# IXarea/LittleGAN

Hardware: AMD Instinct MI355X
Metric: 128x128 CelebA-shaped images/sec (G+D+Adj step) (higher is better)
Workload: dtype bf16; 1 GPU; C3: 128x128x3 synthetic CelebA, batch 256/GPU, bf16 MFMA conv/transposed-conv + Adjuster branch; global_batch=256, per_gpu_batch=256, image=128, cond_dim=40, parallelism=dp1, launch=eager launches

## Files before the change

littlegan_amd/csrc/conv_down3.hip:

```cpp
#include <type_traits>
#include "lg_internal.h"

namespace {

constexpr int TH = 8, TW = 16;
constexpr int HH = 2 * TH + 3;
constexpr int ROWB = 48;
constexpr int KC = 16;
constexpr int NTAP = 25;
template <bool PAIR>
struct D3L {
  static constexpr int HWH = PAIR ? 10 : 18, HWP = PAIR ? 43 : 2 * HWH;
  static constexpr int NROWS = HH * HWP;
  static constexpr int HB = NROWS * ROWB;
  static constexpr int NPIECE = NROWS * 2;
  static constexpr int PPT = (NPIECE + 255) / 256;
  static constexpr int SRED_OFF = 2 * HB;
  static constexpr int SBIAS_OFF = 2 * HB + 256;
  static constexpr int LDS_BYTES = 2 * HB + 256 + 512;
};
#ifndef LG_D3_DBG
#define LG_D3_DBG 0
#endif
constexpr int DBG = LG_D3_DBG;
constexpr int RING = 10;
constexpr int ADEPTH = 2;
constexpr int STAGGER = 6;
constexpr int BLOCKS_PER_CU = 2;

struct D3Params {
  const __bf16* src;
  const char* wp;
  const float* bias;
  __bf16* out;
  double* spart;
  int B, Hs, Ws, Cs, Hm, Wm, N, N32, KB;
  int tpi_x, tpi, ntn, nitems, nparts;
  LgNormFuse nf;
  const float* nstats;
  float nalpha;
  const __bf16* gsrc;
  const float* bcoef;
  unsigned long long* clk;
};

__device__ __forceinline__ int pix32(int r) {
  const int q = r >> 2, lo = r & 3;
  const int odd = (q ^ (q >> 1) ^ (q >> 2)) & 1;
  const int rank = odd ? ((q == 1) ? 0 : (q == 2) ? 1 : (q == 4) ? 2 : 3) : ((q == 0) ? 0 : (q == 3) ? 1 : (q == 5) ? 2 : 3);
  return odd * 16 + rank * 4 + lo;
}

template <bool PAIR>
constexpr int toff_bytes(int t) {
  return ((t / 5) * D3L<PAIR>::HWP + ((t % 5) >> 1) + ((t % 5) & 1) * D3L<PAIR>::HWH) * ROWB;
}

template <bool STATS, bool FUSE = false, bool PAIR = false, int NW = 128, int NORM = 0>
__global__ __launch_bounds__(256, 2) void conv_down3_kernel(const D3Params p) {
  static_assert(!(STATS && FUSE), "forward moments and backward sums are never needed together");
  static_assert(NORM != 1 || (STATS && NW == 128 && !PAIR), "the normalising form exists for the forward passes with fused moments, 8 x 16 tiles");
  static_assert(NORM != 2 || (!STATS && !PAIR && NW == 64), "the backward-normalising form exists for the 64-column data gradients on 8 x 16 tiles");
  static_assert(NW == 128 || (NW == 64 && !PAIR), "tile widths");
  constexpr int NWV = NW / 32, NI = NW / 32;
  constexpr int PPR = NW / 8, NQ = 128 * PPR / 256;
  using L = D3L<PAIR>;
  constexpr int HWH = L::HWH, HWP = L::HWP, HB = L::HB, NPIECE = L::NPIECE, PPT = L::PPT, SRED_OFF = L::SRED_OFF, SBIAS_OFF = L::SBIAS_OFF;
  extern __shared__ __attribute__((aligned(16))) char smem[];
  double* sred = reinterpret_cast<double*>(smem + SRED_OFF);
  const int tid = threadIdx.x, lane = tid & 63, r = lane & 31, h = lane >> 5;
  const int wid = __builtin_amdgcn_readfirstlane(tid >> 6);
  const int wn = wid % NWV, wm = wid / NWV;
  const int G = gridDim.x;
  const int nchunk = p.Cs / KC;
  const int nx = G < 8 ? G : 8, xcd = (int)blockIdx.x % nx, xidx = (int)blockIdx.x / nx;
  const int lb = lg_xcd_remap(blockIdx.x, G);
  const int nfull = p.nitems / G, nrem = p.nitems - nfull * G;
  const int rcnt = (nrem - xcd + nx - 1) / nx;
  const int rstart = nfull * G + xcd * (nrem / nx) + (xcd < nrem % nx ? xcd : nrem % nx);
  const int nmine = nfull + (xidx < rcnt ? 1 : 0);
  const int total = nmine * nchunk;
  const unsigned long long clk_t0 = __builtin_amdgcn_s_memtime(), clk_r0 = __builtin_amdgcn_s_memrealtime();
  int pl[PPT], pyx[PPT];
#pragma unroll
  for (int u = 0; u < PPT; ++u) {
    const int q = tid + u * 256;
    if constexpr (PAIR) {
      pl[u] = -1; pyx[u] = 0;
      if (q < NPIECE) {
        const int row = q >> 1, hy = row / HWP, hxp = row - hy * HWP;
        pl[u] = row * ROWB + (q & 1) * 16;
        const int sm = hxp >= 24, j2 = hxp - 24 * sm, odd = j2 >= HWH, hx = 2 * (j2 - odd * HWH) + odd;
        pyx[u] = (hxp < 20 || hxp >= 24) && hx < 2 * 8 + 3 ? (hy << 8) | (sm << 7) | hx : (0x7fff << 8);
      }
    } else {
      constexpr int PPROW = 2 * (2 * TW + 3);
      pl[u] = -1; pyx[u] = (0x7fff << 8);
      if (q < HH * PPROW) {
        const int hy = q / PPROW, rem = q - hy * PPROW, hx = rem >> 1;
        const int hxp = (hx & 1) ? HWH + (hx >> 1) : (hx >> 1);
        pl[u] = (hy * HWP + hxp) * ROWB + (rem & 1) * 16;
        pyx[u] = (hy << 8) | hx;
      }
    }
  }
  const int half8 = (tid & 1) * 8;

  int abase[NI];
#pragma unroll
  for (int i = 0; i < NI; ++i) {
    const int m = (wm * NI + i) * 32 + pix32(r);
    const int col = m & 15;
    abase[i] = (2 * (m >> 4) * HWP + (PAIR ? col + 16 * (col >> 3) : col)) * ROWB + h * 16;
  }

  struct Item { int n, y0, x0, tn; };
  auto decode = [&](int k) {
    const int item = k == nfull ? rstart + xidx : lb + k * G;
    Item it;
    it.tn = item % p.ntn;
    const int tm = item / p.ntn;
    if constexpr (PAIR) { it.n = 2 * tm; it.y0 = 0; it.x0 = 0; return it; }
    it.n = tm / p.tpi;
    const int tt = tm - it.n * p.tpi;
    it.y0 = (tt / p.tpi_x) * TH; it.x0 = (tt % p.tpi_x) * TW;
    return it;
  };
  constexpr unsigned OOB = 0x80000000u;
  const int sample_elems = p.Hs * p.Ws * p.Cs;
  unsigned hoff[PPT];
  float nmu0 = 0.f, nml0 = 0.f, nna0 = 0.f, nnb0 = 0.f;
  LgBwdCoef bco{};
  auto set_item = [&](const Item& it) __attribute__((always_inline)) {
    if constexpr (NORM == 1) {
      const lg_const_f32p sp = lg_as_const(p.nstats + (long long)it.n * 8);
      nmu0 = lg_uniform(sp[0]); nna0 = lg_uniform(sp[2]); nnb0 = lg_uniform(sp[3]); nml0 = lg_uniform(sp[4]);
    }
    if constexpr (NORM == 2) {
      const lg_const_f32p sp = lg_as_const(p.bcoef + (long long)it.n * 8);
      bco.mu = lg_uniform(sp[0]); bco.mul = lg_uniform(sp[1]); bco.a = lg_uniform(sp[2]); bco.b = lg_uniform(sp[3]);
      bco.m1 = lg_uniform(sp[4]); bco.m2 = lg_uniform(sp[5]); bco.m1l = lg_uniform(sp[6]); bco.m2l = lg_uniform(sp[7]);
    }
#pragma unroll
    for (int u = 0; u < PPT; ++u) {
      const int sy = 2 * it.y0 - 1 + (pyx[u] >> 8), sx = 2 * it.x0 - 1 + (pyx[u] & (PAIR ? 127 : 255));
      const int sl = PAIR ? (pyx[u] >> 7) & 1 : 0;
      const bool ok = pl[u] >= 0 && (unsigned)sy < (unsigned)p.Hs && (unsigned)sx < (unsigned)p.Ws;
      hoff[u] = ok ? (unsigned)((((sl * p.Hs + sy) * p.Ws + sx) * p.Cs + half8) * 2) : OOB;
    }
  };
  auto issue = [&](const Item& it, int c0, u32x4 (&v)[PPT]) __attribute__((always_inline)) {
    const __amdgpu_buffer_rsrc_t rs = __builtin_amdgcn_make_buffer_rsrc(
        const_cast<__bf16*>(p.src + (long long)it.n * sample_elems), 0, (PAIR ? 2 : 1) * sample_elems * 2, 0x00027000);
#pragma unroll
    for (int u = 0; u < PPT; ++u) v[u] = __builtin_bit_cast(u32x4, __builtin_amdgcn_raw_buffer_load_b128(rs, hoff[u] + (unsigned)c0 * 2u, 0, 0));
  };
  auto issue_g = [&](const Item& it, int c0, u32x4 (&v)[NORM == 2 ? PPT : 1]) __attribute__((always_inline)) {
    if constexpr (NORM == 2) {
      const __amdgpu_buffer_rsrc_t rs = __builtin_amdgcn_make_buffer_rsrc(
          const_cast<__bf16*>(p.gsrc + (long long)it.n * sample_elems), 0, sample_elems * 2, 0x00027000);
#pragma unroll
      for (int u = 0; u < PPT; ++u) v[u] = __builtin_bit_cast(u32x4, __builtin_amdgcn_raw_buffer_load_b128(rs, hoff[u] + (unsigned)c0 * 2u, 0, 0));
    }
  };
  u32x4 gv[NORM == 2 ? PPT : 1];
  auto commit = [&](char* buf, const u32x4 (&v)[PPT]) __attribute__((always_inline)) {
#pragma unroll
    for (int u = 0; u < PPT; ++u)
      if (pl[u] >= 0) {
        u32x4 w = v[u];
        if constexpr (NORM == 2) {
          const u32x4 dn = lg_bwdnorm8(w, gv[u], bco, p.nalpha);
          const bool inside = hoff[u] != OOB;
#pragma unroll
          for (int k = 0; k < 4; ++k) w[k] = inside ? dn[k] : 0u;
        }
        if constexpr (NORM == 1) {
          const u32x4 hn = lg_norm8(w, nmu0, nml0, nna0, nnb0, p.nalpha);
          const bool inside = hoff[u] != OOB;
#pragma unroll
          for (int k = 0; k < 4; ++k) w[k] = inside ? hn[k] : 0u;
        }
        if constexpr ((DBG & 16) != 0) {
          const float mu = p.nf.alpha, mul = 0.001f, na = 1.01f, nb = 0.02f, al = 0.3f;
#pragma unroll
          for (int k = 0; k < 4; ++k) {
            float t0 = __builtin_bit_cast(float, w[k] << 16), t1 = __builtin_bit_cast(float, w[k] & 0xffff0000u);
            t0 = na * ((t0 - mu) - mul) + nb; t1 = na * ((t1 - mu) - mul) + nb;
            t0 = fmaxf(t0, al * t0); t1 = fmaxf(t1, al * t1);
            const __bf16 h0 = (__bf16)t0, h1 = (__bf16)t1;
            const unsigned o = (unsigned)__builtin_bit_cast(unsigned short, h0) | ((unsigned)__builtin_bit_cast(unsigned short, h1) << 16);
            w[k] = pyx[u] != (0x7fff << 8) ? o : 0u;
          }
        }
        *reinterpret_cast<u32x4*>(buf + pl[u]) = w;
      }
  };
  const unsigned lane16 = lane * 16;
  const unsigned wstride = (unsigned)p.N32 * (unsigned)p.KB * 1024u;
  auto wbase = [&](int tn, int kb) {
    return p.wp + ((long long)(tn * NWV + wn) * p.KB + kb) * 1024;
  };
  auto wfrag = [&](const char* base, int t) {
    return *reinterpret_cast<const u32x4*>((base + (unsigned long long)t * wstride) + lane16);
  };

  f32x16 acc[NI];
#pragma unroll
  for (int i = 0; i < NI; ++i)
#pragma unroll
    for (int e = 0; e < 16; ++e) acc[i][e] = 0.f;
  static_assert(NTAP % RING != 0, "the slice body is instantiated for the two ring offsets 0 and NTAP % RING");
  constexpr int AD = ADEPTH;
  u32x4 bf[RING];
  u32x4 hv[PPT];

  Item cur = decode(0);
  set_item(cur);
  issue(cur, 0, hv);
  issue_g(cur, 0, gv);
#pragma unroll
  for (int t = 0; t < RING; ++t) bf[t] = wfrag(wbase(cur.tn, 0), t);
  commit(smem, hv);
  __syncthreads();

  float* sbias = reinterpret_cast<float*>(smem + SBIAS_OFF);
  auto load_bias = [&](int tn) {
    if (tid < NW) sbias[tid] = p.bias ? p.bias[tn * NW + tid] : 0.f;
  };
  load_bias(cur.tn);
  {
    if ((int)blockIdx.x >= (G + 1) / 2)
      for (int i = 0; i < STAGGER; ++i) __builtin_amdgcn_s_sleep(16);
  }
  int k = 0, c = 0;
  auto slice = [&](auto off_c, int s) {
    constexpr int OFF = decltype(off_c)::value;
    const bool more = s + 1 < total;
    const bool last_c = c + 1 == nchunk;
    Item nxt = cur;
    int c2 = c + 1;
    if (last_c) { c2 = 0; if (more) { nxt = decode(k + 1); set_item(nxt); } }
    if (!more) c2 = c;
    if constexpr (!(DBG & 4)) { issue(nxt, c2 * KC, hv); issue_g(nxt, c2 * KC, gv); }
    const char* hbuf = smem + (s & 1) * HB;
    const char* wcur = wbase(cur.tn, c);
    const char* wnxt = wbase(nxt.tn, c2);
    bf16x8 a[AD][NI];
#pragma unroll
    for (int d = 0; d + 1 < AD; ++d)
#pragma unroll
      for (int i = 0; i < NI; ++i) a[d][i] = *reinterpret_cast<const bf16x8*>(hbuf + abase[i] + toff_bytes<PAIR>(d));
    __builtin_amdgcn_sched_barrier(0);
#pragma unroll
    for (int t = 0; t < NTAP; ++t) {
      if (t + AD - 1 < NTAP) {
#pragma unroll
        for (int i = 0; i < NI; ++i)
          a[(t + AD - 1) % AD][i] = *reinterpret_cast<const bf16x8*>(hbuf + abase[i] + toff_bytes<PAIR>(t + AD - 1 < NTAP ? t + AD - 1 : 0));
      }
      const int slot = (t + OFF) % RING;
#pragma unroll
      for (int i = 0; i < NI; ++i)
        if constexpr (!(DBG & 1)) acc[i] = __builtin_amdgcn_mfma_f32_32x32x16_bf16(__builtin_bit_cast(bf16x8, bf[slot]), a[t % AD][i], acc[i], 0, 0, 0);
      if constexpr (!(DBG & 2)) {
        if (t + RING < NTAP) bf[slot] = wfrag(wcur, t + RING);
        else bf[slot] = wfrag(wnxt, t + RING - NTAP);
      }
#pragma unroll
      for (int i = 0; i < NI; ++i) {
        __builtin_amdgcn_sched_group_barrier(0x008, 1, 0);
        __builtin_amdgcn_sched_group_barrier(0x100, 1, 0);
      }
      __builtin_amdgcn_sched_group_barrier(0x020, 1, 0);
    }
    if constexpr (NORM != 0) __builtin_amdgcn_sched_barrier(0);
    commit(smem + ((s + 1) & 1) * HB, hv);
    __syncthreads();

    if (last_c && !(DBG & 8)) {
      char* C = smem + (s & 1) * HB;
      const float shift = STATS ? sbias[0] : 0.f;
      const f32x2 shift2 = {shift, shift};
      f32x2 s1v = {0.f, 0.f}, s2v = {0.f, 0.f};
      f32x4 bq[4];
#pragma unroll
      for (int g = 0; g < 4; ++g) bq[g] = *reinterpret_cast<const f32x4*>(sbias + wn * 32 + 8 * g + 4 * h);
#pragma unroll
      for (int i = 0; i < NI; ++i) {
        const int row = (wm * NI + i) * 32 + pix32(r);
#pragma unroll
        for (int g = 0; g < 4; ++g) {
          bf16x4 w;
#pragma unroll
          for (int jj = 0; jj < 2; ++jj) {
            const f32x2 v = f32x2{acc[i][4 * g + 2 * jj], acc[i][4 * g + 2 * jj + 1]} + f32x2{bq[g][2 * jj], bq[g][2 * jj + 1]};
            if constexpr (STATS) {
              const f32x2 d = v - shift2;
              s1v += d;
              s2v = __builtin_elementwise_fma(d, d, s2v);
            }
            w[2 * jj] = (__bf16)v[0]; w[2 * jj + 1] = (__bf16)v[1];
          }
          *reinterpret_cast<bf16x4*>(C + row * (NW * 2) + (((wn * 4 + g) ^ (row & (PPR - 1))) << 4) + 8 * h) = w;
        }
      }
      if constexpr (STATS) {
        const double l1 = (double)s1v[0] + (double)s1v[1], l2 = (double)s2v[0] + (double)s2v[1];
        if constexpr (PAIR) {
          const bool sb = (pix32(r) & 8) != 0;
          const double a1 = lg_wave_sum_d(sb ? 0.0 : l1), a2 = lg_wave_sum_d(sb ? 0.0 : l2);
          const double b1 = lg_wave_sum_d(sb ? l1 : 0.0), b2 = lg_wave_sum_d(sb ? l2 : 0.0);
          if (lane == 0) {
            double* q = sred + (k & 1) * 16;
            q[wid] = a1; q[4 + wid] = a2; q[8 + wid] = b1; q[12 + wid] = b2;
          }
        } else {
          const double w1 = lg_wave_sum_d(l1), w2 = lg_wave_sum_d(l2);
          if (lane == 0) { sred[(k & 1) * 16 + wid] = w1; sred[(k & 1) * 16 + 4 + wid] = w2; }
        }
      }
      const long long obase = ((long long)(cur.n * p.Hm + cur.y0) * p.Wm + cur.x0) * p.N + cur.tn * NW;
      auto pix_off = [&](int row) -> long long {
        if constexpr (PAIR) return obase + (long long)(((row >> 3) & 1) * 64 + (row >> 4) * 8 + (row & 7)) * p.N;
        else return obase + ((long long)(row >> 4) * p.Wm + (row & 15)) * p.N;
      };
      u32x4 zq[FUSE ? NQ : 1];
      (void)zq;
      if constexpr (FUSE) {
#pragma unroll
        for (int q8 = 0; q8 < NQ; ++q8) {
          const int piece = tid + q8 * 256, row = piece / PPR, j = piece % PPR;
          zq[q8] = *reinterpret_cast<const u32x4*>(p.nf.z + pix_off(row) + j * 8);
        }
      }
      __syncthreads();
      float nf1 = 0.f, nf2 = 0.f;
      (void)nf1; (void)nf2;
#pragma unroll
      for (int q8 = 0; q8 < NQ; ++q8) {
        const int piece = tid + q8 * 256, row = piece / PPR, j = piece % PPR;
        const u32x4 v = *reinterpret_cast<const u32x4*>(C + row * (NW * 2) + ((j ^ (row & (PPR - 1))) << 4));
        const long long goff = pix_off(row) + j * 8;
        *reinterpret_cast<u32x4*>(p.out + goff) = v;
        if constexpr (FUSE) {
          const lg_const_f32p sp = lg_as_const(p.nf.stats + (long long)(cur.n + (PAIR ? wid >> 1 : 0)) * 8);
          lg_nf_accum(v, zq[q8], lg_uniform(sp[0]), lg_uniform(sp[4]), lg_uniform(sp[2]), lg_uniform(sp[3]), p.nf.alpha, nf1, nf2);
        }
      }
      if constexpr (FUSE) {
        const double w1 = lg_wave_sum_d((double)nf1), w2 = lg_wave_sum_d((double)nf2);
        if (lane == 0) { sred[(k & 1) * 16 + wid] = w1; sred[(k & 1) * 16 + 4 + wid] = w2; }
      }
      if constexpr (STATS) {
        if (tid == 0) {
          const double* q = sred + (k & 1) * 16;
          if constexpr (PAIR) {
            constexpr double cnt = 64.0 * 128.0;
#pragma unroll
            for (int sm = 0; sm < 2; ++sm) {
              const double S1 = (q[8 * sm] + q[8 * sm + 1]) + (q[8 * sm + 2] + q[8 * sm + 3]);
              const double S2 = (q[8 * sm + 4] + q[8 * sm + 5]) + (q[8 * sm + 6] + q[8 * sm + 7]);
              const double md = S1 / cnt;
              double* o = p.spart + ((long long)(cur.n + sm) * p.nparts + cur.tn) * 3;
              o[0] = cnt; o[1] = (double)shift + md; o[2] = S2 - cnt * md * md;
            }
          } else {
            constexpr double cnt = 128.0 * NW;
            const double S1 = (q[0] + q[1]) + (q[2] + q[3]), S2 = (q[4] + q[5]) + (q[6] + q[7]);
            const double md = S1 / cnt;
            const int tin = (cur.y0 / TH) * p.tpi_x + cur.x0 / TW;
            double* o = p.spart + ((long long)cur.n * p.nparts + tin * p.ntn + cur.tn) * 3;
            o[0] = cnt; o[1] = (double)shift + md; o[2] = S2 - cnt * md * md;
          }
        }
      }
      __syncthreads();
      if constexpr (FUSE) {
        if (tid == 0) {
          const double* q = sred + (k & 1) * 16;
          if constexpr (PAIR) {
#pragma unroll
            for (int sm = 0; sm < 2; ++sm) {
              double* o = p.nf.part + ((long long)(cur.n + sm) * p.nparts + cur.tn) * 2;
              o[0] = q[2 * sm] + q[2 * sm + 1]; o[1] = q[4 + 2 * sm] + q[4 + 2 * sm + 1];
            }
          } else {
            const int tin = (cur.y0 / TH) * p.tpi_x + cur.x0 / TW;
            double* o = p.nf.part + ((long long)cur.n * p.nparts + tin * p.ntn + cur.tn) * 2;
            o[0] = (q[0] + q[1]) + (q[2] + q[3]); o[1] = (q[4] + q[5]) + (q[6] + q[7]);
          }
        }
      }
#pragma unroll
      for (int i = 0; i < NI; ++i)
#pragma unroll
        for (int e = 0; e < 16; ++e) acc[i][e] = 0.f;
      if (more && nxt.tn != cur.tn) load_bias(nxt.tn);
      ++k;
    }
    cur = nxt;
    c = c2;
  };
  for (int s = 0; s < total; s += 2) {
    slice(std::integral_constant<int, 0>{}, s);
    if (s + 1 < total) slice(std::integral_constant<int, NTAP % RING>{}, s + 1);
  }
  if (p.clk && wid == 0 && lane == 0) {
    const unsigned long long t1 = __builtin_amdgcn_s_memtime(), r1 = __builtin_amdgcn_s_memrealtime();
    if (t1 > clk_t0 && r1 > clk_r0) {
      atomicAdd(p.clk, t1 - clk_t0); atomicAdd(p.clk + 1, r1 - clk_r0); atomicAdd(p.clk + 2, 1ull);
    }
  }
}

}

enum D3Tiling { D3_NONE = 0, D3_PLAIN, D3_PAIR, D3_N64 };
static D3Tiling down3_tiling(int B, int Hm, int Wm, int Cs, int N) {
  static int off = -1;
  if (off < 0) off = lg_env_flag("LG_NO_DOWN3") ? 1 : 0;
  if (off || B <= 0 || Cs % KC) return D3_NONE;
  if ((long long)4 * Hm * Wm * Cs * 2 * 2 >= (1ll << 31)) return D3_NONE;
  const bool pair = Hm == 8 && Wm == 8 && B % 2 == 0;
  if (!pair && (Hm % TH || Wm % TW)) return D3_NONE;
  if (N % 128 == 0) return pair ? D3_PAIR : D3_PLAIN;
  return (N % 64 == 0 && !pair) ? D3_N64 : D3_NONE;
}
extern "C" int lg_conv_down3_supported(int B, int Hm, int Wm, int Cs, int N) { return down3_tiling(B, Hm, Wm, Cs, N) != D3_NONE ? 1 : 0; }
extern "C" int lg_conv_down3_zn_supported(int B, int Hm, int Wm, int Cs, int N) {
  return (!lg_env_flag("LG_NO_D3_NORM") && down3_tiling(B, Hm, Wm, Cs, N) == D3_PLAIN) ? 1 : 0;
}
extern "C" int lg_conv_down3_bn_supported(int B, int Hm, int Wm, int Cs, int N) {
  return (!lg_env_flag("LG_NO_D3_BWDNORM") && N == 64 && down3_tiling(B, Hm, Wm, Cs, N) == D3_N64) ? 1 : 0;
}

static int down3_launch(const void* src16, const void* wpack, const float* bias, void* out16, int B, int Hm, int Wm, int Cs, int N,
                        void* spart, size_t spart_bytes, int* nparts_out, const LgNormFuse* nf, size_t nf_bytes,
                        const float* nstats, float nalpha, void* stream, const void* g16 = nullptr, const float* bcoef = nullptr) {
  if (nparts_out) *nparts_out = 0;
  const D3Tiling tiling = down3_tiling(B, Hm, Wm, Cs, N);
  if (tiling == D3_NONE || !src16 || !wpack || !out16) return LG_ERR_UNSUPPORTED;
  const bool pair = tiling == D3_PAIR, n64 = tiling == D3_N64;
  D3Params p{};
  p.src = (const __bf16*)src16; p.wp = (const char*)wpack; p.bias = bias; p.out = (__bf16*)out16;
  p.B = B; p.Hm = Hm; p.Wm = Wm; p.Hs = 2 * Hm; p.Ws = 2 * Wm; p.Cs = Cs; p.N = N; p.N32 = N / 32; p.KB = Cs / 16;
  p.tpi_x = pair ? 1 : Wm / TW; p.tpi = pair ? 1 : p.tpi_x * (Hm / TH); p.ntn = n64 ? N / 64 : N / 128;
  const long long nitems = (long long)(pair ? B / 2 : B) * p.tpi * p.ntn;
  if (nitems <= 0 || nitems >= (1ll << 30)) return LG_ERR_UNSUPPORTED;
  p.nitems = (int)nitems; p.nparts = p.tpi * p.ntn;
  const bool fuse = nf && nf->z && nf->stats && nf->part && nparts_out && (size_t)B * p.nparts * 2 * sizeof(double) <= nf_bytes;
  const bool stats = !fuse && spart && nparts_out && (size_t)B * p.nparts * 3 * sizeof(double) <= spart_bytes;
  if (!nf && spart && nparts_out && !stats) return LG_ERR_UNSUPPORTED;
  p.spart = stats ? (double*)spart : nullptr;
  if (fuse) p.nf = *nf;
  if (nstats && (!stats || n64 || pair)) return LG_ERR_UNSUPPORTED;
  if (g16 && (!fuse || pair || nstats || !n64 || p.ntn != 1)) return LG_ERR_UNSUPPORTED;
  p.nstats = nstats; p.nalpha = nalpha;
  p.gsrc = (const __bf16*)g16; p.bcoef = bcoef;
  p.clk = lg_clock_census();
  static bool attr_set = false;
  if (!attr_set) {
    attr_set = true;
    (void)hipFuncSetAttribute(reinterpret_cast<const void*>(conv_down3_kernel<true>), hipFuncAttributeMaxDynamicSharedMemorySize, D3L<false>::LDS_BYTES);
    (void)hipFuncSetAttribute(reinterpret_cast<const void*>(conv_down3_kernel<false>), hipFuncAttributeMaxDynamicSharedMemorySize, D3L<false>::LDS_BYTES);
    (void)hipFuncSetAttribute(reinterpret_cast<const void*>((conv_down3_kernel<false, true>)), hipFuncAttributeMaxDynamicSharedMemorySize, D3L<false>::LDS_BYTES);
    (void)hipFuncSetAttribute(reinterpret_cast<const void*>((conv_down3_kernel<true, false, true>)), hipFuncAttributeMaxDynamicSharedMemorySize, D3L<true>::LDS_BYTES);
    (void)hipFuncSetAttribute(reinterpret_cast<const void*>((conv_down3_kernel<false, false, true>)), hipFuncAttributeMaxDynamicSharedMemorySize, D3L<true>::LDS_BYTES);
    (void)hipFuncSetAttribute(reinterpret_cast<const void*>((conv_down3_kernel<false, true, true>)), hipFuncAttributeMaxDynamicSharedMemorySize, D3L<true>::LDS_BYTES);
    (void)hipFuncSetAttribute(reinterpret_cast<const void*>((conv_down3_kernel<true, false, false, 64>)), hipFuncAttributeMaxDynamicSharedMemorySize, D3L<false>::LDS_BYTES);
    (void)hipFuncSetAttribute(reinterpret_cast<const void*>((conv_down3_kernel<false, false, false, 64>)), hipFuncAttributeMaxDynamicSharedMemorySize, D3L<false>::LDS_BYTES);
    (void)hipFuncSetAttribute(reinterpret_cast<const void*>((conv_down3_kernel<false, true, false, 64>)), hipFuncAttributeMaxDynamicSharedMemorySize, D3L<false>::LDS_BYTES);
    (void)hipFuncSetAttribute(reinterpret_cast<const void*>((conv_down3_kernel<true, false, false, 128, 1>)), hipFuncAttributeMaxDynamicSharedMemorySize, D3L<false>::LDS_BYTES);
    (void)hipFuncSetAttribute(reinterpret_cast<const void*>((conv_down3_kernel<false, true, false, 64, 2>)), hipFuncAttributeMaxDynamicSharedMemorySize, D3L<false>::LDS_BYTES);
  }
  const int nblk = BLOCKS_PER_CU * lg_grid_cus();
  const int grid = p.nitems < nblk ? p.nitems : nblk;
  hipStream_t st = (hipStream_t)stream;
  constexpr int LDS0 = D3L<false>::LDS_BYTES, LDS1 = D3L<true>::LDS_BYTES;
  if (nstats) {
    hipLaunchKernelGGL((conv_down3_kernel<true, false, false, 128, 1>), dim3(grid), dim3(256), LDS0, st, p);
  } else if (g16) {
    hipLaunchKernelGGL((conv_down3_kernel<false, true, false, 64, 2>), dim3(grid), dim3(256), LDS0, st, p);
  } else if (pair) {
    if (fuse) hipLaunchKernelGGL((conv_down3_kernel<false, true, true>), dim3(grid), dim3(256), LDS1, st, p);
    else if (stats) hipLaunchKernelGGL((conv_down3_kernel<true, false, true>), dim3(grid), dim3(256), LDS1, st, p);
    else hipLaunchKernelGGL((conv_down3_kernel<false, false, true>), dim3(grid), dim3(256), LDS1, st, p);
  } else if (n64) {
    if (fuse) hipLaunchKernelGGL((conv_down3_kernel<false, true, false, 64>), dim3(grid), dim3(256), LDS0, st, p);
    else if (stats) hipLaunchKernelGGL((conv_down3_kernel<true, false, false, 64>), dim3(grid), dim3(256), LDS0, st, p);
    else hipLaunchKernelGGL((conv_down3_kernel<false, false, false, 64>), dim3(grid), dim3(256), LDS0, st, p);
  } else if (fuse) hipLaunchKernelGGL((conv_down3_kernel<false, true>), dim3(grid), dim3(256), LDS0, st, p);
  else if (stats) hipLaunchKernelGGL(conv_down3_kernel<true>, dim3(grid), dim3(256), LDS0, st, p);
  else hipLaunchKernelGGL(conv_down3_kernel<false>, dim3(grid), dim3(256), LDS0, st, p);
  LG_CHECK_LAUNCH("lg_conv_down3");
  lg_note_kernel(g16 ? "conv_down3_kernel<NW=64,BWDNORM>" : nstats ? "conv_down3_kernel<NW=128,NORM>" : pair ? "conv_down3_kernel<PAIR>" : n64 ? "conv_down3_kernel<NW=64>" : "conv_down3_kernel<NW=128>");
  if (stats || fuse) *nparts_out = p.nparts;
  return LG_OK;
}

extern "C" int lg_conv_down3_nf_try(const void* src16, const void* wpack, const float* bias, void* out16, int B, int Hm, int Wm,
                                    int Cs, int N, void* spart, size_t spart_bytes, int* nparts_out, const LgNormFuse* nf,
                                    size_t nf_bytes, void* stream) {
  return down3_launch(src16, wpack, bias, out16, B, Hm, Wm, Cs, N, spart, spart_bytes, nparts_out, nf, nf_bytes, nullptr, 0.f, stream);
}
extern "C" int lg_conv_down3_try(const void* src16, const void* wpack, const float* bias, void* out16, int B, int Hm, int Wm,
                                 int Cs, int N, void* spart, size_t spart_bytes, int* nparts_out, void* stream) {
  return lg_conv_down3_nf_try(src16, wpack, bias, out16, B, Hm, Wm, Cs, N, spart, spart_bytes, nparts_out, nullptr, 0, stream);
}
extern "C" int lg_conv_down3_zn_try(const void* z16, const float* zstats, float alpha, const void* wpack, const float* bias, void* out16,
                                    int B, int Hm, int Wm, int Cs, int N, void* spart, size_t spart_bytes, int* nparts_out, void* stream) {
  if (nparts_out) *nparts_out = 0;
  if (!zstats || !spart || !nparts_out || !lg_conv_down3_zn_supported(B, Hm, Wm, Cs, N)) return LG_ERR_UNSUPPORTED;
  return down3_launch(z16, wpack, bias, out16, B, Hm, Wm, Cs, N, spart, spart_bytes, nparts_out, nullptr, 0, zstats, alpha, stream);
}
extern "C" int lg_conv_down3_bn_try(const void* z16, const void* g16, const float* bcoef, float alpha, const void* wpack, void* out16,
                                    int B, int Hm, int Wm, int Cs, int N, int* nparts_out, const LgNormFuse* nf, size_t nf_bytes,
                                    void* stream) {
  if (nparts_out) *nparts_out = 0;
  if (!g16 || !bcoef || !nf || !nparts_out || !lg_conv_down3_bn_supported(B, Hm, Wm, Cs, N)) return LG_ERR_UNSUPPORTED;
  return down3_launch(z16, wpack, nullptr, out16, B, Hm, Wm, Cs, N, nullptr, 0, nparts_out, nf, nf_bytes, nullptr, alpha, stream, g16, bcoef);
}
```

littlegan_amd/csrc/lg_common.h:

```cpp
#pragma once
#include <hip/hip_runtime.h>
#include <stdint.h>
#include "../../include/littlegan_hip.h"

typedef float f32x4 __attribute__((ext_vector_type(4)));
typedef float f32x2 __attribute__((ext_vector_type(2)));
typedef float f32x16 __attribute__((ext_vector_type(16)));
typedef __bf16 bf16x8 __attribute__((ext_vector_type(8)));
typedef __bf16 bf16x4 __attribute__((ext_vector_type(4)));
typedef short s16x4 __attribute__((ext_vector_type(4)));
typedef unsigned int u32x4 __attribute__((ext_vector_type(4)));

#define LG_NSTAT 8
#define LG_IN_EPS 1e-3f

extern "C" void lg_set_error(const char* fmt, ...);
extern "C" void lg_note_kernel(const char* name);
extern "C" unsigned long long* lg_clock_census(void);

extern "C" int lg_env_flag(const char* name);
extern "C" int lg_halo_enabled(void);
extern "C" int lg_n3_enabled(void);

#define LG_CHECK_ARG(cond, ...)            \
  do {                                     \
    if (!(cond)) {                         \
      lg_set_error(__VA_ARGS__);           \
      return LG_ERR_ARG;                   \
    }                                      \
  } while (0)

#define LG_CHECK_LAUNCH(name)                                              \
  do {                                                                     \
    hipError_t e__ = hipGetLastError();                                    \
    if (e__ != hipSuccess) {                                               \
      lg_set_error("%s: launch failed: %s", name, hipGetErrorString(e__)); \
      return LG_ERR_LAUNCH;                                                \
    }                                                                      \
  } while (0)

__device__ __forceinline__ int lg_xcd_remap(int bid, int nblk) {
  const int q = nblk >> 3, r = nblk & 7;
  const int xcd = bid & 7, idx = bid >> 3;
  const int base = (xcd < r) ? xcd * (q + 1) : r * (q + 1) + (xcd - r) * q;
  return base + idx;
}

__device__ __forceinline__ float lg_leaky(float x, float a) { return x > 0.f ? x : a * x; }

__device__ __forceinline__ float lg_wave_sum(float v) {
#pragma unroll
  for (int o = 32; o > 0; o >>= 1) v += __shfl_xor(v, o, 64);
  return v;
}
__device__ __forceinline__ double lg_wave_sum_d(double v) {
#pragma unroll
  for (int o = 32; o > 0; o >>= 1) v += __shfl_xor(v, o, 64);
  return v;
}

template <int NV>
__device__ __forceinline__ void lg_block_sum(float (&v)[NV], float* smem ) {
  const int lane = threadIdx.x & 63, wid = threadIdx.x >> 6, nw = blockDim.x >> 6;
#pragma unroll
  for (int i = 0; i < NV; ++i) v[i] = lg_wave_sum(v[i]);
  __syncthreads();
  if (lane == 0) {
#pragma unroll
    for (int i = 0; i < NV; ++i) smem[i * 16 + wid] = v[i];
  }
  __syncthreads();
  if (threadIdx.x == 0) {
#pragma unroll
    for (int i = 0; i < NV; ++i) {
      float s = 0.f;
      for (int w = 0; w < nw; ++w) s += smem[i * 16 + w];
      v[i] = s;
    }
  }
}

template <int NV>
__device__ __forceinline__ void lg_block_sum_d(double (&v)[NV], double* smem) {
  const int lane = threadIdx.x & 63, wid = threadIdx.x >> 6, nw = blockDim.x >> 6;
#pragma unroll
  for (int i = 0; i < NV; ++i) v[i] = lg_wave_sum_d(v[i]);
  __syncthreads();
  if (lane == 0) {
#pragma unroll
    for (int i = 0; i < NV; ++i) smem[i * 16 + wid] = v[i];
  }
  __syncthreads();
  if (threadIdx.x == 0) {
#pragma unroll
    for (int i = 0; i < NV; ++i) {
      double s = 0.0;
      for (int w = 0; w < nw; ++w) s += smem[i * 16 + w];
      v[i] = s;
    }
  }
}

struct LgNormFuse {
  const __bf16* z;
  const float* stats;
  double* part;
  float alpha;
  int nparts;
};
__device__ __forceinline__ u32x4 lg_norm8(const u32x4 z8, float mu, float mul, float a, float b, float alpha) {
  u32x4 o;
#pragma unroll
  for (int k = 0; k < 4; ++k) {
    float t0 = __builtin_bit_cast(float, z8[k] << 16), t1 = __builtin_bit_cast(float, z8[k] & 0xffff0000u);
    t0 = a * ((t0 - mu) - mul) + b; t1 = a * ((t1 - mu) - mul) + b;
    t0 = lg_leaky(t0, alpha); t1 = lg_leaky(t1, alpha);
    typedef __bf16 lg_bf16x2 __attribute__((ext_vector_type(2)));
    o[k] = __builtin_bit_cast(unsigned, __builtin_convertvector(f32x2{t0, t1}, lg_bf16x2));
  }
  return o;
}

typedef const float __attribute__((address_space(4)))* lg_const_f32p;
__device__ __forceinline__ lg_const_f32p lg_as_const(const float* p) { return (lg_const_f32p)(p); }
__device__ __forceinline__ float lg_uniform(float x) { return __builtin_bit_cast(float, __builtin_amdgcn_readfirstlane(__builtin_bit_cast(int, x))); }

struct LgBwdCoef { float mu, mul, a, b, m1, m2, m1l, m2l; };
__device__ __forceinline__ u32x4 lg_bwdnorm8(const u32x4 z8, const u32x4 g8, const LgBwdCoef& co, float alpha) {
  u32x4 o;
  typedef __bf16 lg_bf16x2_ __attribute__((ext_vector_type(2)));
#pragma unroll
  for (int k = 0; k < 4; ++k) {
    const float z0 = __builtin_bit_cast(float, z8[k] << 16), z1 = __builtin_bit_cast(float, z8[k] & 0xffff0000u);
    const float g0 = __builtin_bit_cast(float, g8[k] << 16), g1 = __builtin_bit_cast(float, g8[k] & 0xffff0000u);
    const float c0 = (z0 - co.mu) - co.mul, c1 = (z1 - co.mu) - co.mul;
    const float p0 = (co.a * c0 + co.b > 0.f) ? g0 : alpha * g0, p1 = (co.a * c1 + co.b > 0.f) ? g1 : alpha * g1;
    const float d0 = co.a * ((((p0 - co.m1) - co.m1l) - c0 * co.m2) - c0 * co.m2l);
    const float d1 = co.a * ((((p1 - co.m1) - co.m1l) - c1 * co.m2) - c1 * co.m2l);
    o[k] = __builtin_bit_cast(unsigned, __builtin_convertvector(f32x2{d0, d1}, lg_bf16x2_));
  }
  return o;
}

__device__ __forceinline__ void lg_nf_accum(const u32x4 g8, const u32x4 z8, float mu, float mul, float a, float b, float alpha,
                                            float& s1, float& s2) {
#pragma unroll
  for (int k = 0; k < 4; ++k) {
    const float g0 = __builtin_bit_cast(float, g8[k] << 16), g1 = __builtin_bit_cast(float, g8[k] & 0xffff0000u);
    const float z0 = __builtin_bit_cast(float, z8[k] << 16), z1 = __builtin_bit_cast(float, z8[k] & 0xffff0000u);
    const float c0 = (z0 - mu) - mul, c1 = (z1 - mu) - mul;
    const float p0 = (a * c0 + b > 0.f) ? g0 : alpha * g0, p1 = (a * c1 + b > 0.f) ? g1 : alpha * g1;
    s1 += p0; s1 += p1;
    s2 = __builtin_fmaf(p0, c0, s2); s2 = __builtin_fmaf(p1, c1, s2);
  }
}

static inline int lg_cdiv(long long a, long long b) { return (int)((a + b - 1) / b); }
```

Baseline: 24660 images/sec.

## Interleave next-slice normalize and LDS commit into the tail of the MFMA tap loop

Splits the staging (normalization plus LDS store) of the next input slice into per-unit pieces and spreads them across the last taps of the MFMA loop, with sched_group_barrier hints that interleave VALU and DS-write work with the MFMAs. Only the NORM==1 path gets the early start by default, at tap 10. The aim is to hide the serialized commit/normalize phase behind matrix work. The cost is more register pressure and scheduling constraints in the hot loop, and pls uses a dummy address for out-of-bounds pieces.

```diff
diff --git a/littlegan_amd/csrc/conv_down3.hip b/littlegan_amd/csrc/conv_down3.hip
--- a/littlegan_amd/csrc/conv_down3.hip
+++ b/littlegan_amd/csrc/conv_down3.hip
@@ -1,7 +1,13 @@
 #include <type_traits>
+#include <utility>
 #include "lg_internal.h"
 
 namespace {
+
+template <int... I, class Fn>
+__device__ __forceinline__ void d3_static_for_(std::integer_sequence<int, I...>, Fn&& fn) { (fn(std::integral_constant<int, I>{}), ...); }
+template <int N, class Fn>
+__device__ __forceinline__ void d3_static_for(Fn&& fn) { d3_static_for_(std::make_integer_sequence<int, N>{}, fn); }
 
 constexpr int TH = 8, TW = 16;
 constexpr int HH = 2 * TH + 3;
@@ -23,6 +29,8 @@
 #define LG_D3_DBG 0
 #endif
 constexpr int DBG = LG_D3_DBG;
+constexpr int d3_t0(int shift, int dflt) { return ((DBG >> shift) & 31) ? ((DBG >> shift) & 31) - 1 : dflt; }
+constexpr int T0_NORM = d3_t0(8, 10), T0_BWDNORM = d3_t0(16, 25), T0_PLAIN = d3_t0(24, 25);
 constexpr int RING = 10;
 constexpr int ADEPTH = 2;
 constexpr int STAGGER = 6;
@@ -196,6 +204,22 @@
         *reinterpret_cast<u32x4*>(buf + pl[u]) = w;
       }
   };
+  constexpr int T0 = NORM == 1 ? T0_NORM : NORM == 2 ? T0_BWDNORM : T0_PLAIN;
+  static_assert(T0 >= 0 && T0 <= NTAP, "T0 = NTAP: commit behind the tap loop");
+  constexpr bool EARLY = T0 < NTAP;
+  constexpr int NLATE = EARLY ? NTAP - T0 : 1, NUNIT = 4 * PPT;
+  constexpr int UVALU = NORM == 2 ? 36 : NORM == 1 ? 18 : 0;
+  int pls[EARLY ? PPT : 1];
+  if constexpr (EARLY) {
+#pragma unroll
+    for (int u = 0; u < PPT; ++u) pls[u] = pl[u] >= 0 ? pl[u] : tid * ROWB + 32;
+  }
+  auto stage_unit = [&](int u, int k, u32x4 (&v)[PPT]) __attribute__((always_inline)) {
+    const bool inside = hoff[u] != OOB;
+    (void)inside; (void)k;
+    if constexpr (NORM == 1) { const unsigned o = lg_norm2(v[u][k], nmu0, nml0, nna0, nnb0, p.nalpha); v[u][k] = inside ? o : 0u; }
+    if constexpr (NORM == 2) { const unsigned o = lg_bwdnorm2(v[u][k], gv[u][k], bco, p.nalpha); v[u][k] = inside ? o : 0u; }
+  };
   const unsigned lane16 = lane * 16;
   const unsigned wstride = (unsigned)p.N32 * (unsigned)p.KB * 1024u;
   auto wbase = [&](int tn, int kb) {
@@ -252,8 +276,7 @@
 #pragma unroll
       for (int i = 0; i < NI; ++i) a[d][i] = *reinterpret_cast<const bf16x8*>(hbuf + abase[i] + toff_bytes<PAIR>(d));
     __builtin_amdgcn_sched_barrier(0);
-#pragma unroll
-    for (int t = 0; t < NTAP; ++t) {
+    auto tap = [&](int t) __attribute__((always_inline)) {
       if (t + AD - 1 < NTAP) {
 #pragma unroll
         for (int i = 0; i < NI; ++i)
@@ -267,6 +290,10 @@
         if (t + RING < NTAP) bf[slot] = wfrag(wcur, t + RING);
         else bf[slot] = wfrag(wnxt, t + RING - NTAP);
       }
+    };
+#pragma unroll
+    for (int t = 0; t < T0; ++t) {
+      tap(t);
 #pragma unroll
       for (int i = 0; i < NI; ++i) {
         __builtin_amdgcn_sched_group_barrier(0x008, 1, 0);
@@ -274,8 +301,32 @@
       }
       __builtin_amdgcn_sched_group_barrier(0x020, 1, 0);
     }
+    if constexpr (EARLY) {
+      char* obuf = smem + ((s + 1) & 1) * HB;
+      d3_static_for<NLATE>([&](auto l_c) __attribute__((always_inline)) {
+        constexpr int l = decltype(l_c)::value, t = T0 + l;
+        constexpr int j0 = (l * NUNIT + NLATE - 1) / NLATE, j1 = ((l + 1) * NUNIT + NLATE - 1) / NLATE;
+        constexpr int nst = j1 / 4 - j0 / 4;
+        constexpr int vpm = ((j1 - j0) * UVALU + NI - 1) / NI;
+        __builtin_amdgcn_sched_barrier(0);
+        tap(t);
+#pragma unroll
+        for (int j = j0; j < j1; ++j) {
+          stage_unit(j >> 2, j & 3, hv);
+          if ((j & 3) == 3) *reinterpret_cast<u32x4*>(obuf + pls[j >> 2]) = hv[j >> 2];
+        }
+#pragma unroll
+        for (int i = 0; i < NI; ++i) {
+          __builtin_amdgcn_sched_group_barrier(0x008, 1, 0);
+          __builtin_amdgcn_sched_group_barrier(0x100, 1, 0);
+          if constexpr (vpm > 0) __builtin_amdgcn_sched_group_barrier(0x002, vpm, 0);
+        }
+        __builtin_amdgcn_sched_group_barrier(0x020, 1, 0);
+        if constexpr (nst > 0) __builtin_amdgcn_sched_group_barrier(0x200, nst, 0);
+      });
+    }
     if constexpr (NORM != 0) __builtin_amdgcn_sched_barrier(0);
-    commit(smem + ((s + 1) & 1) * HB, hv);
+    if constexpr (!EARLY) commit(smem + ((s + 1) & 1) * HB, hv);
     __syncthreads();
 
     if (last_c && !(DBG & 8)) {
diff --git a/littlegan_amd/csrc/lg_common.h b/littlegan_amd/csrc/lg_common.h
--- a/littlegan_amd/csrc/lg_common.h
+++ b/littlegan_amd/csrc/lg_common.h
@@ -108,16 +108,17 @@
   float alpha;
   int nparts;
 };
+__device__ __forceinline__ unsigned lg_norm2(const unsigned z2, float mu, float mul, float a, float b, float alpha) {
+  float t0 = __builtin_bit_cast(float, z2 << 16), t1 = __builtin_bit_cast(float, z2 & 0xffff0000u);
+  t0 = a * ((t0 - mu) - mul) + b; t1 = a * ((t1 - mu) - mul) + b;
+  t0 = lg_leaky(t0, alpha); t1 = lg_leaky(t1, alpha);
+  typedef __bf16 lg_bf16x2 __attribute__((ext_vector_type(2)));
+  return __builtin_bit_cast(unsigned, __builtin_convertvector(f32x2{t0, t1}, lg_bf16x2));
+}
 __device__ __forceinline__ u32x4 lg_norm8(const u32x4 z8, float mu, float mul, float a, float b, float alpha) {
   u32x4 o;
 #pragma unroll
-  for (int k = 0; k < 4; ++k) {
-    float t0 = __builtin_bit_cast(float, z8[k] << 16), t1 = __builtin_bit_cast(float, z8[k] & 0xffff0000u);
-    t0 = a * ((t0 - mu) - mul) + b; t1 = a * ((t1 - mu) - mul) + b;
-    t0 = lg_leaky(t0, alpha); t1 = lg_leaky(t1, alpha);
-    typedef __bf16 lg_bf16x2 __attribute__((ext_vector_type(2)));
-    o[k] = __builtin_bit_cast(unsigned, __builtin_convertvector(f32x2{t0, t1}, lg_bf16x2));
-  }
+  for (int k = 0; k < 4; ++k) o[k] = lg_norm2(z8[k], mu, mul, a, b, alpha);
   return o;
 }
 
@@ -126,19 +127,20 @@
 __device__ __forceinline__ float lg_uniform(float x) { return __builtin_bit_cast(float, __builtin_amdgcn_readfirstlane(__builtin_bit_cast(int, x))); }
 
 struct LgBwdCoef { float mu, mul, a, b, m1, m2, m1l, m2l; };
+__device__ __forceinline__ unsigned lg_bwdnorm2(const unsigned z2, const unsigned g2, const LgBwdCoef& co, float alpha) {
+  typedef __bf16 lg_bf16x2_ __attribute__((ext_vector_type(2)));
+  const float z0 = __builtin_bit_cast(float, z2 << 16), z1 = __builtin_bit_cast(float, z2 & 0xffff0000u);
+  const float g0 = __builtin_bit_cast(float, g2 << 16), g1 = __builtin_bit_cast(float, g2 & 0xffff0000u);
+  const float c0 = (z0 - co.mu) - co.mul, c1 = (z1 - co.mu) - co.mul;
+  const float p0 = (co.a * c0 + co.b > 0.f) ? g0 : alpha * g0, p1 = (co.a * c1 + co.b > 0.f) ? g1 : alpha * g1;
+  const float d0 = co.a * ((((p0 - co.m1) - co.m1l) - c0 * co.m2) - c0 * co.m2l);
+  const float d1 = co.a * ((((p1 - co.m1) - co.m1l) - c1 * co.m2) - c1 * co.m2l);
+  return __builtin_bit_cast(unsigned, __builtin_convertvector(f32x2{d0, d1}, lg_bf16x2_));
+}
 __device__ __forceinline__ u32x4 lg_bwdnorm8(const u32x4 z8, const u32x4 g8, const LgBwdCoef& co, float alpha) {
   u32x4 o;
-  typedef __bf16 lg_bf16x2_ __attribute__((ext_vector_type(2)));
 #pragma unroll
-  for (int k = 0; k < 4; ++k) {
-    const float z0 = __builtin_bit_cast(float, z8[k] << 16), z1 = __builtin_bit_cast(float, z8[k] & 0xffff0000u);
-    const float g0 = __builtin_bit_cast(float, g8[k] << 16), g1 = __builtin_bit_cast(float, g8[k] & 0xffff0000u);
-    const float c0 = (z0 - co.mu) - co.mul, c1 = (z1 - co.mu) - co.mul;
-    const float p0 = (co.a * c0 + co.b > 0.f) ? g0 : alpha * g0, p1 = (co.a * c1 + co.b > 0.f) ? g1 : alpha * g1;
-    const float d0 = co.a * ((((p0 - co.m1) - co.m1l) - c0 * co.m2) - c0 * co.m2l);
-    const float d1 = co.a * ((((p1 - co.m1) - co.m1l) - c1 * co.m2) - c1 * co.m2l);
-    o[k] = __builtin_bit_cast(unsigned, __builtin_convertvector(f32x2{d0, d1}, lg_bf16x2_));
-  }
+  for (int k = 0; k < 4; ++k) o[k] = lg_bwdnorm2(z8[k], g8[k], co, alpha);
   return o;
 }
 
```

Result: no change. 24650 images/sec (-0.0%).
